# WangFeng18/3d-gaussian-splatting

Hardware: AMD Instinct MI355X
Metric: render_fps (higher is better)
Workload: dtype f32; 1 GPU; cfg5: 2400000 Gaussians, 1920x1080, no SH, forward render, one frame in flight, one view per GPU -- north-star target scene (geometry of BASELINE configs[3]/[4]); n_gaussians=2400000, visible=1887982, tile_pairs=6950364, width=1920, height=1080, parallelism=view-sharded x1 (no data-path collective), frames_in_flight=1

## Files before the change

### 3d-gaussian-splatting_amd/csrc/cull_project.hip

```cpp
#include <atomic>
#include <mutex>

#include "gs_common.h"
#include "gs_frame_layout.h"
#include "project_common.h"
#include "strip_common.h"
#include "tile_bin_common.h"

namespace {

__global__ void __launch_bounds__(256) global_culling_kernel(
    const float *__restrict__ pos, const float4 *__restrict__ quat, const float *__restrict__ scale,
    const float *__restrict__ rot, const float *__restrict__ tran, int64_t n, float near_plane,
    float half_w, float half_h, float *__restrict__ res_pos, float4 *__restrict__ res_cov,
    int64_t *__restrict__ mask) {
    Cam cam;
#pragma unroll
    for (int i = 0; i < 9; ++i) cam.rot[i] = rot[i];
#pragma unroll
    for (int i = 0; i < 3; ++i) cam.tran[i] = tran[i];
    for (int64_t pid = (int64_t)blockIdx.x * blockDim.x + threadIdx.x; pid < n;
         pid += (int64_t)gridDim.x * blockDim.x) {
        float p[3], s[3], pi[3], cv[4];
        load3(pos, pid, p);
// ... 170 lines not shown
    vis = 0;
    cxy = make_float2(0.f, 0.f);
    uint2 rc = make_uint2(0, 0);
    float depth = 0.f;
    if (project_cull(in.p, P.cam, P.near_plane, P.half_w, P.half_h, pc, pi)) {
        project_cov_static(pc, in.RSSR, P.cam, pi, cv);
        vis = 1;
        uint32_t y0, y1, x0, x1;
        cnt = P.cull_method == 0 ? dist_rect(pi[0], pi[1], P, y0, y1, x0, x1)
                                 : tile_rect(pi[0], pi[1], cv, P, y0, y1, x0, x1);
        rc = make_uint2(y0 | (y1 << 16), x0 | (x1 << 16));
        depth = pi[2];
        cxy = make_float2(pi[0], pi[1]);
        const float4 col = make_float4(in.col[0], in.col[1], in.col[2], 0.0f);
        float cA = 0.f, cB = 0.f, cC = 0.f;
        gs_conic(cv[0], cv[1], cv[2], cv[3], cA, cB, cC);
        float4 *rec = rec_geom + pid * GS_REC_STRIDE;
        rec[0] = make_float4(pi[0], pi[1], pi[2], in.opa_act);
        rec[1] = make_float4(cv[0], cv[1], cv[2], cv[3]);
        rec[2] = col;
        rec[3] = make_float4(cA, cB, cC, 0.f);
    }
    if (tiles_touched) tiles_touched[pid] = cnt;
    const uint4 out = make_uint4(rc.x, rc.y, __float_as_uint(depth), cnt);
    rects[pid] = out;
    return out;
}
__device__ __forceinline__ uint4 project_one(const RawGaussian &in, int64_t pid, const ProjectParams &P,
                                             float4 *__restrict__ rec_geom, uint32_t *__restrict__ tiles_touched,
                                             uint4 *__restrict__ rects, uint32_t &vis, float2 &cxy) {
    return project_one(make_static(in, P.scale_act, P.color_dim), pid, P, rec_geom, tiles_touched, rects, vis, cxy);
}

__global__ void __launch_bounds__(256) scene_pack_build_kernel(
    const float *__restrict__ pos, const float4 *__restrict__ quat, const float *__restrict__ scale,
    const float *__restrict__ opa, const float *__restrict__ rgb, int64_t n, int scale_act, int color_dim,
    float4 *__restrict__ pack_a, float4 *__restrict__ pack_b) {
    for (int64_t pid = (int64_t)blockIdx.x * blockDim.x + threadIdx.x; pid < n; pid += (int64_t)gridDim.x * blockDim.x) {
        float s[3];
        const StaticGaussian g = make_static(load_raw(pos, quat, scale, opa, rgb, pid, color_dim), scale_act, color_dim, s);
        float smax = fmaxf(s[0], fmaxf(s[1], s[2]));
        if (!(s[0] + s[1] + s[2] < 3.0e38f)) smax = __uint_as_float(0x7fc00000u);
        pack_a[pid] = make_float4(g.p[0], g.p[1], g.p[2], smax);
        store_static(pack_b, pid, g);
    }
}

__global__ void __launch_bounds__(256) frame_project_kernel(
    const float *__restrict__ pos, const float4 *__restrict__ quat, const float *__restrict__ scale,
    const float *__restrict__ opa, const float *__restrict__ rgb, int64_t n, ProjectParams P,
    float4 *__restrict__ rec_geom,
    uint32_t *__restrict__ tiles_touched, uint4 *__restrict__ rects, uint32_t *__restrict__ block_sums,
    uint32_t *__restrict__ block_vis) {
    const int64_t pid = (int64_t)blockIdx.x * blockDim.x + threadIdx.x;
    uint32_t cnt = 0, vis = 0;
    if (pid < n) {
        float2 cxy;
        cnt = project_one(load_raw(pos, quat, scale, opa, rgb, pid, P.color_dim), pid, P, rec_geom, tiles_touched, rects,
                          vis, cxy).w;
    }
    __shared__ uint32_t s_cnt[4], s_vis[4];
    uint32_t wsum = gs_wave_sum_u32(cnt), wvis = gs_wave_sum_u32(vis);
    const int wave = threadIdx.x >> 6;
    if ((threadIdx.x & 63) == 0) {
        s_cnt[wave] = wsum;
        s_vis[wave] = wvis;
    }
    __syncthreads();
    if (threadIdx.x == 0) {
        block_sums[blockIdx.x] = s_cnt[0] + s_cnt[1] + s_cnt[2] + s_cnt[3];
        block_vis[blockIdx.x] = s_vis[0] + s_vis[1] + s_vis[2] + s_vis[3];
    }
}

template <bool DIST, bool PACKED>
__device__ __forceinline__ void project_count_body(
    const float *__restrict__ pos, const float4 *__restrict__ quat, const float *__restrict__ scale,
    const float *__restrict__ opa, const float *__restrict__ rgb, const float4 *__restrict__ pack_b, int64_t n, ProjectParams P,
    float4 *__restrict__ rec_geom, uint32_t *__restrict__ tiles_touched, uint4 *__restrict__ rects, GsDistCull D,
    uint32_t per_slice, gs_strip_geom SG, uint32_t S, uint32_t slice0, unsigned long long *__restrict__ table,
    uint32_t *__restrict__ slice_pairs, uint32_t *__restrict__ slice_vis, const uint32_t *__restrict__ tile_cost,
    uint32_t n_tiles, uint32_t *__restrict__ tile_order, const unsigned long long *__restrict__ gate) {
    extern __shared__ unsigned long long s_hist[];
    __shared__ uint32_t s_acc[2];
    if (gate && *gate == 0) return;
    if (blockIdx.x >= S) {
        tile_order_workgroup(tile_cost, n_tiles, tile_order);
        return;
    }
    const uint32_t slice = slice0 + strip_slice_of_block(blockIdx.x, S);
    const int64_t g0 = (int64_t)slice * per_slice;
    auto in_range = [&](uint32_t i) { return i < per_slice && g0 + i < n; };
    auto load = [&](int64_t pid) {
        if constexpr (PACKED) return load_static(pack_b, pid);
        else return load_raw(pos, quat, scale, opa, rgb, pid, P.color_dim);
    };
    decltype(load(0)) cur = {}, nxt = {};
    if (in_range(threadIdx.x)) cur = load(g0 + threadIdx.x);
    for (uint32_t t = threadIdx.x; t < SG.NS; t += STRIP_THREADS) s_hist[t] = 0;
    if (threadIdx.x < 2) s_acc[threadIdx.x] = 0;
    __syncthreads();
    settle(cur);
    uint32_t acc_cnt = 0, acc_vis = 0;
    for (uint32_t base = 0; base < per_slice; base += STRIP_THREADS) {
        const uint32_t i = base + threadIdx.x;
        if (in_range(i + STRIP_THREADS)) nxt = load(g0 + i + STRIP_THREADS);
        uint4 rc = make_uint4(0, 0, 0, 0);
        uint32_t vis = 0;
        float2 cxy = make_float2(0.f, 0.f);
        if (in_range(i)) rc = project_one(cur, g0 + i, P, rec_geom, tiles_touched, rects, vis, cxy);
        acc_cnt += rc.w;
        acc_vis += vis;
        walk_strips<DIST>(rc, g0 + i, SG, cxy, D,
                          [&](uint32_t strip, uint32_t, uint32_t, uint32_t np) { atomicAdd(&s_hist[strip], (1ull << 32) | np); });
        cur = nxt;
    }
    acc_cnt = gs_wave_sum_u32(acc_cnt);
    acc_vis = gs_wave_sum_u32(acc_vis);
    if ((threadIdx.x & 63) == 0) {
        atomicAdd(&s_acc[0], acc_cnt);
        atomicAdd(&s_acc[1], acc_vis);
    }
    __syncthreads();
    unsigned long long *row = table + (size_t)slice * SG.NS;
    for (uint32_t t = threadIdx.x; t < SG.NS; t += STRIP_THREADS) row[t] = s_hist[t];
    if (threadIdx.x == 0) {
        slice_pairs[slice] = s_acc[0];
        slice_vis[slice] = s_acc[1];
    }
}

template <bool DIST>
__global__ void __launch_bounds__(STRIP_THREADS) frame_project_count_kernel(
    const float *__restrict__ pos, const float4 *__restrict__ quat, const float *__restrict__ scale,
    const float *__restrict__ opa, const float *__restrict__ rgb, int64_t n, ProjectParams P,
    float4 *__restrict__ rec_geom, uint32_t *__restrict__ tiles_touched, uint4 *__restrict__ rects, GsDistCull D,
    uint32_t per_slice, gs_strip_geom SG, uint32_t S, uint32_t slice0, unsigned long long *__restrict__ table,
    uint32_t *__restrict__ slice_pairs, uint32_t *__restrict__ slice_vis, const uint32_t *__restrict__ tile_cost,
    uint32_t n_tiles, uint32_t *__restrict__ tile_order, const unsigned long long *__restrict__ gate) {
    project_count_body<DIST, false>(pos, quat, scale, opa, rgb, nullptr, n, P, rec_geom, tiles_touched, rects, D, per_slice, SG, S, slice0, table, slice_pairs, slice_vis,
                                    tile_cost, n_tiles, tile_order, gate);
}
template <bool DIST>
__global__ void __launch_bounds__(STRIP_THREADS) frame_packed_project_count_kernel(
    const float4 *__restrict__ pack_b, int64_t n, ProjectParams P,
    float4 *__restrict__ rec_geom, uint32_t *__restrict__ tiles_touched, uint4 *__restrict__ rects, GsDistCull D,
    uint32_t per_slice, gs_strip_geom SG, uint32_t S, uint32_t slice0, unsigned long long *__restrict__ table,
    uint32_t *__restrict__ slice_pairs, uint32_t *__restrict__ slice_vis, const uint32_t *__restrict__ tile_cost,
    uint32_t n_tiles, uint32_t *__restrict__ tile_order, const unsigned long long *__restrict__ gate) {
    project_count_body<DIST, true>(nullptr, nullptr, nullptr, nullptr, nullptr, pack_b, n, P, rec_geom, tiles_touched, rects, D, per_slice, SG, S, slice0, table, slice_pairs, slice_vis,
                                    tile_cost, n_tiles, tile_order, gate);
}

#define GS_OCC_QCAP 16384u
#define GS_OCC_LEVELS 4
struct OccPyramid {
    const uint32_t *t0;
    uint32_t o1, o2, o3;
    uint32_t st0, d1, d2, d3;
};
__device__ __forceinline__ bool occluded_everywhere(const float pi[3], float z, float smax, uint32_t dbits,
                                                    const ProjectParams &P, const OccPyramid &Y) {
    if (P.cull_method != 2) return false;
    const float k = P.occ_k * smax * gs_rcp(z);
    const float ax = 1.0f + pi[0] * pi[0], ay = 1.0f + pi[1] * pi[1];
    const float rx = k * (ax * gs_rsq(ax)) * 1.0001f, ry = k * (ay * gs_rsq(ay)) * 1.0001f;
    const float fx0 = (pi[0] - rx - P.leftmost) * P.inv_tlx - 1e-3f, fx1 = (pi[0] + rx - P.leftmost) * P.inv_tlx + 1e-3f;
    const float fy0 = (pi[1] - ry - P.topmost) * P.inv_tly - 1e-3f, fy1 = (pi[1] + ry - P.topmost) * P.inv_tly + 1e-3f;
    if (!(fx1 - fx0 < 16.0f) || !(fy1 - fy0 < 16.0f)) return false;
    if (fx1 < 0.f || fy1 < 0.f) return true;
    uint32_t x0 = gs_f2u_sat(fx0), y0 = gs_f2u_sat(fy0), x1 = gs_f2u_sat(fx1), y1 = gs_f2u_sat(fy1);
    if (x0 >= P.ntx || y0 >= P.nty) return true;
    x1 = x1 < P.ntx ? x1 : P.ntx - 1;
    y1 = y1 < P.nty ? y1 : P.nty - 1;
    const uint32_t e = (x1 - x0) > (y1 - y0) ? (x1 - x0) : (y1 - y0);
    const uint32_t L = e <= 1 ? 0u : (e <= 3 ? 1u : (e <= 7 ? 2u : 3u));
    const uint32_t m1 = L >= 1 ? ~0u : 0u, m2 = L >= 2 ? ~0u : 0u, m3 = L >= 3 ? ~0u : 0u;
    const uint32_t *tab = Y.t0 + ((Y.o1 & m1) + (Y.o2 & m2) + (Y.o3 & m3));
    const uint32_t st = Y.st0 + ((Y.d1 & m1) + (Y.d2 & m2) + (Y.d3 & m3));
    const uint32_t cx0 = x0 >> L, cy0 = y0 >> L, w = (x1 >> L) - cx0, h = (y1 >> L) - cy0;
    uint32_t m = 0;
#pragma unroll
    for (uint32_t j = 0; j < 3; ++j)
#pragma unroll
        for (uint32_t i = 0; i < 3; ++i) {
            const uint32_t c = tab[(cy0 + (j < h ? j : h)) * st + cx0 + (i < w ? i : w)];
            m = c > m ? c : m;
        }
    return dbits > m;
}

template <bool PACKED>
__device__ __forceinline__ void project_cull_count_body(
    const float *__restrict__ pos, const float4 *__restrict__ quat, const float *__restrict__ scale,
    const float *__restrict__ opa, const float *__restrict__ rgb, const float4 *__restrict__ pack_a,
    const float4 *__restrict__ pack_b, int64_t n, ProjectParams P,
    float4 *__restrict__ rec_geom, uint4 *__restrict__ rects, uint32_t per_slice, gs_strip_geom SG, uint32_t S,
    unsigned long long *__restrict__ table, uint32_t *__restrict__ slice_pairs, uint32_t *__restrict__ slice_vis,
    const uint32_t *__restrict__ tile_cost, uint32_t n_tiles, uint32_t *__restrict__ tile_order,
    const uint32_t *__restrict__ cut, uint32_t qcap, uint32_t stash_cap, unsigned long long *__restrict__ stage_ent,
    uint32_t *__restrict__ stage_tag, uint32_t ecap, uint32_t *__restrict__ slice_entries) {
    extern __shared__ unsigned long long s_hist[];
    __shared__ uint32_t s_acc[2], s_qn, s_ne;
    if (blockIdx.x >= S) {
        tile_order_workgroup(tile_cost, n_tiles, tile_order);
        return;
    }
    const uint32_t slice = strip_slice_of_block(blockIdx.x, S);
    const int64_t g0 = (int64_t)slice * per_slice;
    const int lane = threadIdx.x & 63;
    uint32_t *s_cut = reinterpret_cast<uint32_t *>(s_hist + SG.NS);
    const uint32_t st0 = SG.nsx * GS_STRIP_W;
    const uint32_t w1 = (SG.ntx + 1) / 2, h1 = (SG.nty + 1) / 2, w2 = (w1 + 1) / 2, h2 = (h1 + 1) / 2, w3 = (w2 + 1) / 2,
                   h3 = (h2 + 1) / 2;
    uint32_t *s_l1 = s_cut + st0 * SG.nty, *s_l2 = s_l1 + w1 * h1, *s_l3 = s_l2 + w2 * h2;
    uint16_t *s_q = reinterpret_cast<uint16_t *>(s_l3 + w3 * h3);
    float *s_stash = reinterpret_cast<float *>(s_q + ((qcap + 1) & ~1u));
    const OccPyramid Y = {s_cut, st0 * SG.nty, w1 * h1, w2 * h2, st0, w1 - st0, w2 - w1, w3 - w2};
    auto fetch_at = [&](float (&pp)[3], float (&ss)[3], uint32_t i) {
        int64_t g = g0 + i;
        g = g < n ? g : n - 1;
        if constexpr (PACKED) {
            const float4 v = pack_a[g];
            pp[0] = v.x; pp[1] = v.y; pp[2] = v.z; ss[0] = v.w;
            ss[1] = ss[2] = 0.f;
        } else {
            load3(pos, g, pp);
            load3(scale, g, ss);
        }
    };
    float pa[3], sa[3], pb[3], sb[3];
    fetch_at(pa, sa, threadIdx.x);
    fetch_at(pb, sb, threadIdx.x + STRIP_THREADS);
    for (uint32_t t = threadIdx.x; t < SG.NS; t += STRIP_THREADS) s_hist[t] = 0;
    for (uint32_t t0 = threadIdx.x; t0 < st0 * SG.nty; t0 += 8 * STRIP_THREADS) {
        uint32_t v[8];
#pragma unroll
        for (uint32_t k = 0; k < 8; ++k) {
            const uint32_t t = t0 + k * STRIP_THREADS, iy = t / st0, ix = t - iy * st0;
            const bool in = iy < SG.nty && ix < SG.ntx;
            v[k] = cut[in ? iy * SG.ntx + ix : 0u];
            v[k] = in ? v[k] : GS_NO_CUT;
        }
#pragma unroll
        for (uint32_t k = 0; k < 8; ++k)
            if (t0 + k * STRIP_THREADS < st0 * SG.nty) s_cut[t0 + k * STRIP_THREADS] = v[k];
    }
    if (threadIdx.x < 2) s_acc[threadIdx.x] = 0;
    if (threadIdx.x == 2) s_ne = 0;
    unsigned long long *const ent = stage_ent + (size_t)slice * ecap;
    uint32_t *const tag = stage_tag + (size_t)slice * ecap;
    auto build = [&](uint32_t *dst, uint32_t dw, uint32_t dh, const uint32_t *src, uint32_t sst, uint32_t sw, uint32_t sh) {
        __syncthreads();
        for (uint32_t t = threadIdx.x; t < dw * dh; t += STRIP_THREADS) {
            const uint32_t cy = t / dw, cx = t - cy * dw, x = 2 * cx, y = 2 * cy;
            uint32_t m = src[y * sst + x];
            if (x + 1 < sw) m = max(m, src[y * sst + x + 1]);
            if (y + 1 < sh) {
                m = max(m, src[(y + 1) * sst + x]);
                if (x + 1 < sw) m = max(m, src[(y + 1) * sst + x + 1]);
            }
            dst[t] = m;
        }
    };
    build(s_l1, w1, h1, s_cut, st0, SG.ntx, SG.nty);
    build(s_l2, w2, h2, s_l1, w1, w1, h1);
    build(s_l3, w3, h3, s_l2, w2, w2, h2);
    uint32_t acc_cnt = 0, acc_vis = 0;
    for (uint32_t c0 = 0; c0 < per_slice; c0 += qcap) {
        const uint32_t cn = per_slice - c0 < qcap ? per_slice - c0 : qcap;
        if (threadIdx.x == 0) s_qn = 0;
        __syncthreads();
        auto in_chunk = [&](uint32_t i) { return i < cn && g0 + c0 + i < n; };
        auto fetch = [&](float (&pp)[3], float (&ss)[3], uint32_t i) { fetch_at(pp, ss, c0 + i); };
        auto test = [&](const float (&pp)[3], const float (&ss)[3], uint32_t i) {
            bool surv = false;
            if (in_chunk(i)) {
                float pc[3], pi[3];
                if (project_cull(pp, P.cam, P.near_plane, P.half_w, P.half_h, pc, pi)) {
                    const float dep = sqrtf(pc[0] * pc[0] + pc[1] * pc[1] + pc[2] * pc[2]);
                    float smax;
                    bool finite;
                    if constexpr (PACKED) {
                        smax = ss[0];
                        finite = smax < 3.0e38f;
                    } else {
                        float s[3];
#pragma unroll
                        for (int k = 0; k < 3; ++k) s[k] = P.scale_act == 0 ? fabsf(ss[k]) + 1e-4f : gs_exp2(GS_LOG2E * ss[k]);
                        smax = fmaxf(s[0], fmaxf(s[1], s[2]));
                        finite = s[0] + s[1] + s[2] < 3.0e38f;
                    }
                    if (finite && occluded_everywhere(pi, pc[2], smax, __float_as_uint(dep), P, Y)) {
                        acc_vis += 1;
                    } else {
                        surv = true;
                    }
                }
            }
            const unsigned long long b = __ballot(surv);
            if (b) {
                uint32_t wbase = 0;
                if (lane == 0) wbase = atomicAdd(&s_qn, (uint32_t)__popcll(b));
                wbase = __shfl(wbase, 0, 64);
                if (surv) {
                    const uint32_t slot = wbase + (uint32_t)__popcll(b & ((1ull << lane) - 1ull));
                    s_q[slot] = (uint16_t)i;
                    if (!PACKED && slot < stash_cap) {
#pragma unroll
                        for (int c = 0; c < 3; ++c) {
                            s_stash[c * stash_cap + slot] = pp[c];
                            s_stash[(3 + c) * stash_cap + slot] = ss[c];
                        }
                    }
                }
            }
        };
        float pq[3], sq[3];
        if (c0 != 0) {
            fetch(pa, sa, threadIdx.x);
            fetch(pb, sb, threadIdx.x + STRIP_THREADS);
        }
        for (uint32_t base = 0; base < cn; base += 3 * STRIP_THREADS) {
            const uint32_t i = base + threadIdx.x;
            fetch(pq, sq, i + 2 * STRIP_THREADS);
            test(pa, sa, i);
            if (base + STRIP_THREADS >= cn) break;
            fetch(pa, sa, i + 3 * STRIP_THREADS);
            test(pb, sb, i + STRIP_THREADS);
            if (base + 2 * STRIP_THREADS >= cn) break;
            fetch(pb, sb, i + 4 * STRIP_THREADS);
            test(pq, sq, i + 2 * STRIP_THREADS);
        }
        __syncthreads();
        const uint32_t nq = s_qn;
        auto load_survivor = [&](uint32_t k, uint32_t q) {
            const int64_t pid = g0 + c0 + q;
            if constexpr (PACKED) {
                return load_static(pack_b, pid);
            } else {
                RawGaussian r;
                if (k < stash_cap) {
#pragma unroll
                    for (int c = 0; c < 3; ++c) {
                        r.p[c] = s_stash[c * stash_cap + k];
                        r.sraw[c] = s_stash[(3 + c) * stash_cap + k];
                    }
                } else {
                    load3(pos, pid, r.p);
                    load3(scale, pid, r.sraw);
                }
                const float4 q4 = quat[pid];
                r.qraw[0] = q4.x; r.qraw[1] = q4.y; r.qraw[2] = q4.z; r.qraw[3] = q4.w;
                r.opa = opa[pid];
                r.rgb[0] = r.rgb[1] = r.rgb[2] = 0.f;
                if (P.color_dim == 3) load3(rgb, pid, r.rgb);
                return r;
            }
        };
        decltype(load_survivor(0, 0)) cur = {}, nxt = {};
        uint32_t qi = 0, qn_ = 0;
        if (threadIdx.x < nq) {
            qi = s_q[threadIdx.x];
            cur = load_survivor(threadIdx.x, qi);
        }
        settle(cur);
        for (uint32_t base = 0; base < nq; base += STRIP_THREADS) {
            const uint32_t k = base + threadIdx.x;
            if (k + STRIP_THREADS < nq) {
                qn_ = s_q[k + STRIP_THREADS];
                nxt = load_survivor(k + STRIP_THREADS, qn_);
            }
            uint4 rc = make_uint4(0, 0, 0, 0);
            uint32_t vis = 0;
            float2 cxy = make_float2(0.f, 0.f);
            const int64_t pid = g0 + c0 + qi;
            if (k < nq) rc = project_one(cur, pid, P, rec_geom, nullptr, rects, vis, cxy);
            acc_cnt += rc.w;
            acc_vis += vis;
            walk_strips<false, true>(rc, pid, SG, cxy, GsDistCull{},
                                     [&](uint32_t strip, uint32_t lo32, uint32_t d, uint32_t np) {
                                         const uint32_t rank = (uint32_t)(atomicAdd(&s_hist[strip], (1ull << 32) | np) >> 32);
                                         const unsigned long long act = __ballot(true);
                                         uint32_t wbase = 0;
                                         if (lane == __ffsll((long long)act) - 1) wbase = atomicAdd(&s_ne, (uint32_t)__popcll(act));
                                         wbase = (uint32_t)__builtin_amdgcn_readfirstlane((int)wbase);
                                         const uint32_t slot = wbase + (uint32_t)__popcll(act & ((1ull << lane) - 1ull));
                                         if (slot < ecap) {
                                             ent[slot] = ((unsigned long long)d << 32) | lo32;
                                             tag[slot] = strip_tag(strip, rank);
                                         }
                                     },
                                     s_cut);
            cur = nxt;
            qi = qn_;
        }
    }
    acc_cnt = gs_wave_sum_u32(acc_cnt);
    acc_vis = gs_wave_sum_u32(acc_vis);
    if (lane == 0) {
        atomicAdd(&s_acc[0], acc_cnt);
        atomicAdd(&s_acc[1], acc_vis);
    }
    __syncthreads();
    const uint32_t ne = s_ne;
    const bool fits = ne <= ecap;
    unsigned long long *row = table + (size_t)slice * SG.NS;
    for (uint32_t t = threadIdx.x; t < SG.NS; t += STRIP_THREADS) row[t] = fits ? s_hist[t] : 0ull;
    if (threadIdx.x == 0) {
        slice_pairs[slice] = s_acc[0];
        slice_vis[slice] = s_acc[1];
        slice_entries[slice] = fits ? ne : GS_STAGE_OVER;
    }
}

__global__ void __launch_bounds__(STRIP_THREADS) frame_project_cull_count_kernel(
    const float *__restrict__ pos, const float4 *__restrict__ quat, const float *__restrict__ scale,
    const float *__restrict__ opa, const float *__restrict__ rgb, int64_t n, ProjectParams P,
    float4 *__restrict__ rec_geom, uint4 *__restrict__ rects, uint32_t per_slice, gs_strip_geom SG, uint32_t S,
    unsigned long long *__restrict__ table, uint32_t *__restrict__ slice_pairs, uint32_t *__restrict__ slice_vis,
    const uint32_t *__restrict__ tile_cost, uint32_t n_tiles, uint32_t *__restrict__ tile_order,
    const uint32_t *__restrict__ cut, uint32_t qcap, uint32_t stash_cap, unsigned long long *__restrict__ stage_ent,
    uint32_t *__restrict__ stage_tag, uint32_t ecap, uint32_t *__restrict__ slice_entries) {
    project_cull_count_body<false>(pos, quat, scale, opa, rgb, nullptr, nullptr, n, P, rec_geom, rects, per_slice, SG, S, table, slice_pairs, slice_vis, tile_cost, n_tiles, tile_order, cut,
                                   qcap, stash_cap, stage_ent, stage_tag, ecap, slice_entries);
}
__global__ void __launch_bounds__(STRIP_THREADS) frame_packed_project_cull_count_kernel(
    const float4 *__restrict__ pack_a, const float4 *__restrict__ pack_b, int64_t n, ProjectParams P,
    float4 *__restrict__ rec_geom, uint4 *__restrict__ rects, uint32_t per_slice, gs_strip_geom SG, uint32_t S,
    unsigned long long *__restrict__ table, uint32_t *__restrict__ slice_pairs, uint32_t *__restrict__ slice_vis,
    const uint32_t *__restrict__ tile_cost, uint32_t n_tiles, uint32_t *__restrict__ tile_order,
    const uint32_t *__restrict__ cut, uint32_t qcap, uint32_t stash_cap, unsigned long long *__restrict__ stage_ent,
    uint32_t *__restrict__ stage_tag, uint32_t ecap, uint32_t *__restrict__ slice_entries) {
    project_cull_count_body<true>(nullptr, nullptr, nullptr, nullptr, nullptr, pack_a, pack_b, n, P, rec_geom, rects, per_slice, SG, S, table, slice_pairs, slice_vis, tile_cost, n_tiles, tile_order, cut,
                                   qcap, stash_cap, stage_ent, stage_tag, ecap, slice_entries);
}

template <bool DIST>
__global__ void __launch_bounds__(BIN_THREADS) frame_project_bin_count_kernel(
    const float *__restrict__ pos, const float4 *__restrict__ quat, const float *__restrict__ scale,
    const float *__restrict__ opa, const float *__restrict__ rgb, int64_t n, ProjectParams P,
    float4 *__restrict__ rec_geom, uint4 *__restrict__ rects, GsDistCull D, uint32_t per_block, uint32_t T,
    uint32_t *__restrict__ table, uint32_t *__restrict__ slice_pairs, uint32_t *__restrict__ slice_vis) {
    extern __shared__ uint32_t s_tile_hist[];
    __shared__ uint32_t s_acc[2];
    const uint32_t slice = slice_of_block(blockIdx.x, gridDim.x);
    const int64_t g0 = (int64_t)slice * per_block;
    auto in_range = [&](uint32_t i) { return i < per_block && g0 + i < n; };
    RawGaussian cur = {}, nxt = {};
    if (in_range(threadIdx.x)) cur = load_raw(pos, quat, scale, opa, rgb, g0 + threadIdx.x, P.color_dim);
    for (uint32_t t = threadIdx.x; t < T; t += BIN_THREADS) s_tile_hist[t] = 0;
    if (threadIdx.x < 2) s_acc[threadIdx.x] = 0;
    __syncthreads();
    settle(cur);
    uint32_t acc_cnt = 0, acc_vis = 0;
    for (uint32_t base = 0; base < per_block; base += BIN_THREADS) {
        const uint32_t i = base + threadIdx.x;
        if (in_range(i + BIN_THREADS)) nxt = load_raw(pos, quat, scale, opa, rgb, g0 + i + BIN_THREADS, P.color_dim);
        uint4 rc = make_uint4(0, 0, 0, 0);
        uint32_t vis = 0;
        float2 cxy = make_float2(0.f, 0.f);
        if (in_range(i)) rc = project_one(cur, g0 + i, P, rec_geom, nullptr, rects, vis, cxy);
        acc_cnt += rc.w;
        acc_vis += vis;
        walk_rect<DIST>(rc, g0 + i, P.ntx, cxy, D, [&](uint32_t tile, uint32_t, uint32_t) { atomicAdd(&s_tile_hist[tile], 1u); });
        cur = nxt;
    }
    acc_cnt = gs_wave_sum_u32(acc_cnt);
    acc_vis = gs_wave_sum_u32(acc_vis);
    if ((threadIdx.x & 63) == 0) {
        atomicAdd(&s_acc[0], acc_cnt);
        atomicAdd(&s_acc[1], acc_vis);
    }
    __syncthreads();
    uint32_t *row = table + (size_t)slice * T;
    for (uint32_t t = threadIdx.x; t < T; t += BIN_THREADS) row[t] = s_tile_hist[t];
    if (threadIdx.x == 0) {
        slice_pairs[slice] = s_acc[0];
        slice_vis[slice] = s_acc[1];
    }
}

}

extern "C" int gs_world2camera(const float *pos, const float *rot, const float *tran, float *res, int64_t B,
                               gs_stream_t stream) {
    GS_CHECK_ARG(B >= 0, "B < 0");
    if (B == 0) return 0;
    GS_CHECK_ARG(pos && rot && tran && res, "null pointer");
    hipLaunchKernelGGL(world2camera_kernel, dim3(grid_for(B, 256)), dim3(256), 0, (hipStream_t)stream, pos, rot,
                       tran, res, B);
    GS_CHECK_LAUNCH();
    return 0;
}

extern "C" int gs_world2camera_backward(const float *grad_out, const float *rot, float *grad_inp, int64_t B,
                                        gs_stream_t stream) {
    GS_CHECK_ARG(B >= 0, "B < 0");
    if (B == 0) return 0;
    GS_CHECK_ARG(grad_out && rot && grad_inp, "null pointer");
    hipLaunchKernelGGL(world2camera_backward_kernel, dim3(grid_for(B, 256)), dim3(256), 0, (hipStream_t)stream,
                       grad_out, rot, grad_inp, B);
    GS_CHECK_LAUNCH();
    return 0;
}

extern "C" int gs_jacobian(const float *pos_cam, float *jac, int64_t B, gs_stream_t stream) {
    GS_CHECK_ARG(B >= 0, "B < 0");
    if (B == 0) return 0;
    GS_CHECK_ARG(pos_cam && jac, "null pointer");
    hipLaunchKernelGGL(jacobian_kernel, dim3(grid_for(B, 256)), dim3(256), 0, (hipStream_t)stream, pos_cam, jac, B);
    GS_CHECK_LAUNCH();
    return 0;
}

extern "C" int gs_global_culling(const float *pos, const float *quat, const float *scale, const float *rot,
                                 const float *tran, int64_t N, float near_plane, float half_width,
                                 float half_height, float *res_pos, float *res_cov, int64_t *culling_mask,
                                 gs_stream_t stream) {
    GS_CHECK_ARG(N >= 0, "N < 0");
    if (N == 0) return 0;
    GS_CHECK_ARG(pos && quat && scale && rot && tran && res_pos && res_cov && culling_mask, "null pointer");
    GS_CHECK_ARG(((uintptr_t)quat & 15) == 0 && ((uintptr_t)res_cov & 15) == 0, "quat/res_cov must be 16-byte aligned");
    hipLaunchKernelGGL(global_culling_kernel, dim3(grid_for(N, 256)), dim3(256), 0, (hipStream_t)stream, pos,
                       (const float4 *)quat, scale, rot, tran, N, near_plane, half_width, half_height, res_pos,
                       (float4 *)res_cov, culling_mask);
    GS_CHECK_LAUNCH();
    return 0;
}

extern "C" size_t gs_scene_pack_bytes(int64_t N, size_t *a_bytes, size_t *b_bytes) {
    const size_t a = N < 0 ? 0 : ((size_t)N * 16 + 255) / 256 * 256, b = N < 0 ? 0 : ((size_t)N * 64 + 255) / 256 * 256;
    if (a_bytes) *a_bytes = a;
    if (b_bytes) *b_bytes = b;
    return a + b;
}

extern "C" int gs_scene_pack_build(const float *pos, const float *quat, const float *scale, const float *opa, const float *rgb,
                                   int64_t N, int32_t color_dim, int32_t scale_activation, void *pack_a, void *pack_b,
                                   gs_stream_t stream) {
    GS_CHECK_ARG(N >= 0 && N < (1ll << 31), "N out of range");
    GS_CHECK_ARG(color_dim == 3 || color_dim == 27 || color_dim == 48, "color_dim must be 3, 27 or 48");
    GS_CHECK_ARG(scale_activation == 0 || scale_activation == 1, "scale_activation must be 0 (abs) or 1 (exp)");
    if (N == 0) return 0;
    GS_CHECK_ARG(pos && quat && scale && opa && rgb && pack_a && pack_b, "null pointer");
    GS_CHECK_ARG(((uintptr_t)quat & 15) == 0, "quat must be 16-byte aligned");
    GS_CHECK_ARG(((uintptr_t)pack_a & 15) == 0 && ((uintptr_t)pack_b & 63) == 0,
                 "pack_a must be 16-byte aligned, pack_b 64-byte aligned");
    hipLaunchKernelGGL(scene_pack_build_kernel, dim3(grid_for(N, 256)), dim3(256), 0, (hipStream_t)stream, pos,
                       (const float4 *)quat, scale, opa, rgb, N, (int)scale_activation, (int)color_dim, (float4 *)pack_a,
                       (float4 *)pack_b);
    GS_CHECK_LAUNCH();
    return 0;
}

int gs_stage_project(const gs_frame *f, const gs_frame_ws &ws, hipStream_t stream, int slice_begin, int slice_end,
                     bool second_pass) {
    ProjectParams P = make_params(f);
    uint32_t *touched = f->sort_mode == 2 && gs_frame_geometry(f).n_tiles <= GS_BIN_MAX_TILES ? nullptr : ws.tiles_touched;
    if (gs_frame_uses_strips(f)) {
        touched = nullptr;
        gs_frame_geom G = gs_frame_geometry(f);
        const gs_strip_plan plan = gs_strip_plan_for(f->N, G.ntx, G.nty);
        const gs_strip_geom SG = plan.geom;
        const GsDistCull D = gs_frame_dist_cull(f);
        static std::mutex attr_mu;
        static std::atomic<uint64_t> attr_done{0};
        int dev = 0;
        GS_HIP(hipGetDevice(&dev));
        if (dev < 64 && !((attr_done.load(std::memory_order_acquire) >> dev) & 1)) {
            std::lock_guard<std::mutex> lock(attr_mu);
            for (const void *fn : {(const void *)frame_project_count_kernel<false>, (const void *)frame_project_count_kernel<true>,
                                   (const void *)frame_packed_project_count_kernel<false>, (const void *)frame_packed_project_count_kernel<true>,
                                   (const void *)frame_project_cull_count_kernel, (const void *)frame_packed_project_cull_count_kernel})
                GS_HIP(hipFuncSetAttribute(fn, hipFuncAttributeMaxDynamicSharedMemorySize, GS_BIN_LDS_BYTES - 8 * 4096));
            attr_done.fetch_or(1ull << dev, std::memory_order_release);
        }
        unsigned long long *table = (unsigned long long *)ws.strip_table;
        if (slice_end < 0) slice_end = (int)plan.slices;
        GS_CHECK_ARG(slice_begin >= 0 && slice_begin < slice_end && slice_end <= (int)plan.slices, "bad slice range");
        const uint32_t nsl = (uint32_t)(slice_end - slice_begin);
        const bool packed = gs_frame_scene_pack(f);
        const float4 *pack_a = packed ? (const float4 *)gs_frame_scene_fields(f)->scene_pack_a : nullptr;
        const float4 *pack_b = packed ? (const float4 *)gs_frame_scene_fields(f)->scene_pack_b : nullptr;
        if (gs_frame_occlusion_cull(f) && !second_pass) {
            GS_CHECK_ARG(slice_begin == 0 && nsl == plan.slices, "an occlusion-culled frame is projected in one piece");
            uint32_t qcap_max = GS_OCC_QCAP;
            if (const char *e = getenv("GS_OCC_QCAP")) {
                const long v = atol(e);
                if (v >= 64 && v <= (long)GS_OCC_QCAP) qcap_max = (uint32_t)v;
            }
            const uint32_t qcap = plan.per_slice < qcap_max ? plan.per_slice : qcap_max;
            size_t lds = sizeof(unsigned long long) * SG.NS + gs_cull_pyramid_bytes(G.ntx, G.nty) + 2 * (size_t)qcap + 16;
            const size_t room = (size_t)GS_BIN_LDS_BYTES - 8 * 4096;
            uint32_t stash_cap = room > lds ? (uint32_t)((room - lds) / 24) & ~63u : 0u;
            if (stash_cap > qcap) stash_cap = (qcap + 63u) & ~63u;
            if (packed) stash_cap = 0;
            if (const char *e = getenv("GS_OCC_STASH")) {
                const long v = atol(e);
                if (v >= 0 && (uint32_t)v < stash_cap) stash_cap = (uint32_t)v & ~63u;
            }
            lds += (size_t)stash_cap * 24;
#define GS_CULL_TAIL                                                                                                   \
    f->N, P, ws.rec_geom, ws.rects, plan.per_slice, SG, nsl, table, ws.slice_pairs, ws.slice_vis, ws.tile_cost,        \
        (uint32_t)G.n_tiles, ws.tile_order, gs_frame_cut_table(f, ws), qcap, stash_cap, (unsigned long long *)ws.keys_b, \
        ws.vals_b, gs_cull_stage_cap(f->max_pairs, plan.slices), ws.slice_entries
            if (packed)
                hipLaunchKernelGGL(frame_packed_project_cull_count_kernel, dim3(nsl + 1), dim3(STRIP_THREADS), lds, stream, pack_a,
                                   pack_b, GS_CULL_TAIL);
            else
                hipLaunchKernelGGL(frame_project_cull_count_kernel, dim3(nsl + 1), dim3(STRIP_THREADS), lds, stream, f->pos,
                                   (const float4 *)f->quat, f->scale, f->opa, f->rgb, GS_CULL_TAIL);
#undef GS_CULL_TAIL
            GS_CHECK_LAUNCH();
            return 0;
        }
        const size_t lds = sizeof(unsigned long long) * SG.NS;
        const uint32_t extra = (slice_begin == 0 && !second_pass) ? 1u : 0u;
        const unsigned long long *gate = second_pass ? ws.counters + GS_CNT_RANPAST : nullptr;
#define GS_COUNT_TAIL                                                                                                  \
    f->N, P, ws.rec_geom, touched, ws.rects, D, plan.per_slice, SG, nsl, (uint32_t)slice_begin, table, ws.slice_pairs, \
        ws.slice_vis, ws.tile_cost, (uint32_t)G.n_tiles, ws.tile_order, gate
#define GS_LAUNCH_PROJECT_COUNT(DIST)                                                                                  \
    do {                                                                                                               \
        if (packed)                                                                                                    \
            hipLaunchKernelGGL(frame_packed_project_count_kernel<DIST>, dim3(nsl + extra), dim3(STRIP_THREADS), lds,   \
                               stream, pack_b, GS_COUNT_TAIL);                                                         \
        else                                                                                                           \
            hipLaunchKernelGGL(frame_project_count_kernel<DIST>, dim3(nsl + extra), dim3(STRIP_THREADS), lds, stream,  \
                               f->pos, (const float4 *)f->quat, f->scale, f->opa, f->rgb, GS_COUNT_TAIL);              \
    } while (0)
        if (f->tile_culling_method == 0)
            GS_LAUNCH_PROJECT_COUNT(true);
        else
            GS_LAUNCH_PROJECT_COUNT(false);
#undef GS_LAUNCH_PROJECT_COUNT
#undef GS_COUNT_TAIL
        GS_CHECK_LAUNCH();
        return 0;
    }
    GS_CHECK_ARG(!second_pass, "the second pass of an occlusion-culled frame belongs to the strip variant's project + count stage");
    GS_CHECK_ARG(slice_begin == 0 && slice_end < 0, "this frame's project stage cannot be issued in ranges");
    if (gs_frame_fused_table_count(f)) {
        gs_frame_geom G = gs_frame_geometry(f);
        const GsDistCull D = gs_frame_dist_cull(f);
        static std::mutex attr_mu2;
        static std::atomic<uint64_t> attr_done2{0};
        int dev = 0;
        GS_HIP(hipGetDevice(&dev));
        if (dev < 64 && !((attr_done2.load(std::memory_order_acquire) >> dev) & 1)) {
            std::lock_guard<std::mutex> lock(attr_mu2);
            for (const void *fn : {(const void *)frame_project_bin_count_kernel<false>, (const void *)frame_project_bin_count_kernel<true>})
                GS_HIP(hipFuncSetAttribute(fn, hipFuncAttributeMaxDynamicSharedMemorySize, GS_BIN_MAX_TILES * 4));
            attr_done2.fetch_or(1ull << dev, std::memory_order_release);
        }
        const uint32_t per_block = bin_per_block(f->N), B = (uint32_t)gs_div_up(f->N, per_block);
        const uint32_t T = (uint32_t)G.n_tiles;
#define GS_LAUNCH_PROJECT_BIN(DIST)                                                                                    \
    hipLaunchKernelGGL(frame_project_bin_count_kernel<DIST>, dim3(B), dim3(BIN_THREADS), sizeof(uint32_t) * T, stream, \
                       f->pos, (const float4 *)f->quat, f->scale, f->opa, f->rgb, f->N, P, ws.rec_geom, ws.rects, D,   \
                       per_block, T, ws.bin_table, ws.slice_pairs, ws.slice_vis)
        if (f->tile_culling_method == 0)
            GS_LAUNCH_PROJECT_BIN(true);
        else
            GS_LAUNCH_PROJECT_BIN(false);
#undef GS_LAUNCH_PROJECT_BIN
        GS_CHECK_LAUNCH();
        return 0;
    }
    int nblk = (int)gs_div_up(f->N, 256);
    hipLaunchKernelGGL(frame_project_kernel, dim3(nblk), dim3(256), 0, stream, f->pos, (const float4 *)f->quat,
                       f->scale, f->opa, f->rgb, f->N, P, ws.rec_geom,
                       touched, ws.rects, ws.block_sums, ws.block_vis);
    GS_CHECK_LAUNCH();
    return 0;
}
```

Measured before the change: 4507 frames/s.

## Stream occlusion-cull survivors through per-wave LDS rings instead of chunked block queue

Replaces the chunked two-phase scheme, where a block tests a chunk, syncs, then projects the queued survivors, with a per-wavefront ring buffer in LDS. Each wave projects 64 survivors as soon as they accumulate, interleaved with culling the next candidates, and leftovers go to a shared tail list that is handled after a single block barrier. The goal is to remove block-wide barriers and idle phases and to overlap cull tests with projection. In exchange, each wave needs its own small parameter stash, sizing becomes more intricate, and correctness depends on ordering the ring within a wavefront.

```diff
diff --git a/3d-gaussian-splatting_amd/csrc/cull_project.hip b/3d-gaussian-splatting_amd/csrc/cull_project.hip
--- a/3d-gaussian-splatting_amd/csrc/cull_project.hip
+++ b/3d-gaussian-splatting_amd/csrc/cull_project.hip
@@ -346,7 +346,6 @@
                                     tile_cost, n_tiles, tile_order, gate);
 }
 
-#define GS_OCC_QCAP 16384u
 #define GS_OCC_LEVELS 4
 struct OccPyramid {
     const uint32_t *t0;
@@ -384,6 +383,9 @@
     return dbits > m;
 }
 
+#define GS_OCC_RING 128u
+#define GS_OCC_TAIL (16u * 63u)
+
 template <bool PACKED>
 __device__ __forceinline__ void project_cull_count_body(
     const float *__restrict__ pos, const float4 *__restrict__ quat, const float *__restrict__ scale,
@@ -392,26 +394,27 @@
     float4 *__restrict__ rec_geom, uint4 *__restrict__ rects, uint32_t per_slice, gs_strip_geom SG, uint32_t S,
     unsigned long long *__restrict__ table, uint32_t *__restrict__ slice_pairs, uint32_t *__restrict__ slice_vis,
     const uint32_t *__restrict__ tile_cost, uint32_t n_tiles, uint32_t *__restrict__ tile_order,
-    const uint32_t *__restrict__ cut, uint32_t qcap, uint32_t stash_cap, unsigned long long *__restrict__ stage_ent,
+    const uint32_t *__restrict__ cut, uint32_t par_slots, unsigned long long *__restrict__ stage_ent,
     uint32_t *__restrict__ stage_tag, uint32_t ecap, uint32_t *__restrict__ slice_entries) {
     extern __shared__ unsigned long long s_hist[];
-    __shared__ uint32_t s_acc[2], s_qn, s_ne;
+    __shared__ uint32_t s_acc[2], s_tn, s_ne;
     if (blockIdx.x >= S) {
         tile_order_workgroup(tile_cost, n_tiles, tile_order);
         return;
     }
     const uint32_t slice = strip_slice_of_block(blockIdx.x, S);
     const int64_t g0 = (int64_t)slice * per_slice;
-    const int lane = threadIdx.x & 63;
+    const uint32_t lane = threadIdx.x & 63, wave = threadIdx.x >> 6;
     uint32_t *s_cut = reinterpret_cast<uint32_t *>(s_hist + SG.NS);
     const uint32_t st0 = SG.nsx * GS_STRIP_W;
     const uint32_t w1 = (SG.ntx + 1) / 2, h1 = (SG.nty + 1) / 2, w2 = (w1 + 1) / 2, h2 = (h1 + 1) / 2, w3 = (w2 + 1) / 2,
                    h3 = (h2 + 1) / 2;
     uint32_t *s_l1 = s_cut + st0 * SG.nty, *s_l2 = s_l1 + w1 * h1, *s_l3 = s_l2 + w2 * h2;
-    uint16_t *s_q = reinterpret_cast<uint16_t *>(s_l3 + w3 * h3);
-    float *s_stash = reinterpret_cast<float *>(s_q + ((qcap + 1) & ~1u));
+    uint32_t *s_tail = s_l3 + w3 * h3 + (STRIP_THREADS / 64) * GS_OCC_RING;
+    uint32_t *const ring = s_l3 + w3 * h3 + wave * GS_OCC_RING;
+    float *const par = reinterpret_cast<float *>(s_tail + GS_OCC_TAIL) + wave * 6 * par_slots;
     const OccPyramid Y = {s_cut, st0 * SG.nty, w1 * h1, w2 * h2, st0, w1 - st0, w2 - w1, w3 - w2};
-    auto fetch_at = [&](float (&pp)[3], float (&ss)[3], uint32_t i) {
+    auto fetch = [&](float (&pp)[3], float (&ss)[3], uint32_t i) {
         int64_t g = g0 + i;
         g = g < n ? g : n - 1;
         if constexpr (PACKED) {
@@ -424,8 +427,8 @@
         }
     };
     float pa[3], sa[3], pb[3], sb[3];
-    fetch_at(pa, sa, threadIdx.x);
-    fetch_at(pb, sb, threadIdx.x + STRIP_THREADS);
+    fetch(pa, sa, threadIdx.x);
+    fetch(pb, sb, threadIdx.x + STRIP_THREADS);
     for (uint32_t t = threadIdx.x; t < SG.NS; t += STRIP_THREADS) s_hist[t] = 0;
     for (uint32_t t0 = threadIdx.x; t0 < st0 * SG.nty; t0 += 8 * STRIP_THREADS) {
         uint32_t v[8];
@@ -442,6 +445,7 @@
     }
     if (threadIdx.x < 2) s_acc[threadIdx.x] = 0;
     if (threadIdx.x == 2) s_ne = 0;
+    if (threadIdx.x == 3) s_tn = 0;
     unsigned long long *const ent = stage_ent + (size_t)slice * ecap;
     uint32_t *const tag = stage_tag + (size_t)slice * ecap;
     auto build = [&](uint32_t *dst, uint32_t dw, uint32_t dh, const uint32_t *src, uint32_t sst, uint32_t sw, uint32_t sh) {
@@ -460,134 +464,168 @@
     build(s_l1, w1, h1, s_cut, st0, SG.ntx, SG.nty);
     build(s_l2, w2, h2, s_l1, w1, w1, h1);
     build(s_l3, w3, h3, s_l2, w2, w2, h2);
+    __syncthreads();
     uint32_t acc_cnt = 0, acc_vis = 0;
-    for (uint32_t c0 = 0; c0 < per_slice; c0 += qcap) {
-        const uint32_t cn = per_slice - c0 < qcap ? per_slice - c0 : qcap;
-        if (threadIdx.x == 0) s_qn = 0;
-        __syncthreads();
-        auto in_chunk = [&](uint32_t i) { return i < cn && g0 + c0 + i < n; };
-        auto fetch = [&](float (&pp)[3], float (&ss)[3], uint32_t i) { fetch_at(pp, ss, c0 + i); };
-        auto test = [&](const float (&pp)[3], const float (&ss)[3], uint32_t i) {
-            bool surv = false;
-            if (in_chunk(i)) {
-                float pc[3], pi[3];
-                if (project_cull(pp, P.cam, P.near_plane, P.half_w, P.half_h, pc, pi)) {
-                    const float dep = sqrtf(pc[0] * pc[0] + pc[1] * pc[1] + pc[2] * pc[2]);
-                    float smax;
-                    bool finite;
-                    if constexpr (PACKED) {
-                        smax = ss[0];
-                        finite = smax < 3.0e38f;
-                    } else {
-                        float s[3];
+    uint32_t head = 0, tail = 0;
+    auto ring_order = [] {
+        __builtin_amdgcn_fence(__ATOMIC_ACQ_REL, "wavefront");
+        __builtin_amdgcn_wave_barrier();
+    };
+    auto in_slice = [&](uint32_t i) { return i < per_slice && g0 + i < n; };
+    auto test = [&](const float (&pp)[3], const float (&ss)[3], uint32_t i) {
+        bool surv = false;
+        if (in_slice(i)) {
+            float pc[3], pi[3];
+            if (project_cull(pp, P.cam, P.near_plane, P.half_w, P.half_h, pc, pi)) {
+                const float dep = sqrtf(pc[0] * pc[0] + pc[1] * pc[1] + pc[2] * pc[2]);
+                float smax;
+                bool finite;
+                if constexpr (PACKED) {
+                    smax = ss[0];
+                    finite = smax < 3.0e38f;
+                } else {
+                    float s[3];
 #pragma unroll
-                        for (int k = 0; k < 3; ++k) s[k] = P.scale_act == 0 ? fabsf(ss[k]) + 1e-4f : gs_exp2(GS_LOG2E * ss[k]);
-                        smax = fmaxf(s[0], fmaxf(s[1], s[2]));
-                        finite = s[0] + s[1] + s[2] < 3.0e38f;
-                    }
-                    if (finite && occluded_everywhere(pi, pc[2], smax, __float_as_uint(dep), P, Y)) {
-                        acc_vis += 1;
-                    } else {
-                        surv = true;
-                    }
+                    for (int k = 0; k < 3; ++k) s[k] = P.scale_act == 0 ? fabsf(ss[k]) + 1e-4f : gs_exp2(GS_LOG2E * ss[k]);
+                    smax = fmaxf(s[0], fmaxf(s[1], s[2]));
+                    finite = s[0] + s[1] + s[2] < 3.0e38f;
+                }
+                if (finite && occluded_everywhere(pi, pc[2], smax, __float_as_uint(dep), P, Y)) {
+                    acc_vis += 1;
+                } else {
+                    surv = true;
                 }
             }
-            const unsigned long long b = __ballot(surv);
-            if (b) {
-                uint32_t wbase = 0;
-                if (lane == 0) wbase = atomicAdd(&s_qn, (uint32_t)__popcll(b));
-                wbase = __shfl(wbase, 0, 64);
-                if (surv) {
-                    const uint32_t slot = wbase + (uint32_t)__popcll(b & ((1ull << lane) - 1ull));
-                    s_q[slot] = (uint16_t)i;
-                    if (!PACKED && slot < stash_cap) {
+        }
+        const unsigned long long b = __ballot(surv);
+        if (surv) {
+            const uint32_t below = __builtin_amdgcn_mbcnt_hi((uint32_t)(b >> 32), __builtin_amdgcn_mbcnt_lo((uint32_t)b, 0u));
+            const uint32_t slot = (tail + below) & (GS_OCC_RING - 1);
+            ring[slot] = i;
+            if (!PACKED && slot < par_slots) {
 #pragma unroll
-                        for (int c = 0; c < 3; ++c) {
-                            s_stash[c * stash_cap + slot] = pp[c];
-                            s_stash[(3 + c) * stash_cap + slot] = ss[c];
-                        }
-                    }
+                for (int c = 0; c < 3; ++c) {
+                    par[c * par_slots + slot] = pp[c];
+                    par[(3 + c) * par_slots + slot] = ss[c];
                 }
             }
-        };
-        float pq[3], sq[3];
-        if (c0 != 0) {
-            fetch(pa, sa, threadIdx.x);
-            fetch(pb, sb, threadIdx.x + STRIP_THREADS);
-        }
-        for (uint32_t base = 0; base < cn; base += 3 * STRIP_THREADS) {
-            const uint32_t i = base + threadIdx.x;
-            fetch(pq, sq, i + 2 * STRIP_THREADS);
-            test(pa, sa, i);
-            if (base + STRIP_THREADS >= cn) break;
-            fetch(pa, sa, i + 3 * STRIP_THREADS);
-            test(pb, sb, i + STRIP_THREADS);
-            if (base + 2 * STRIP_THREADS >= cn) break;
-            fetch(pb, sb, i + 4 * STRIP_THREADS);
-            test(pq, sq, i + 2 * STRIP_THREADS);
-        }
-        __syncthreads();
-        const uint32_t nq = s_qn;
-        auto load_survivor = [&](uint32_t k, uint32_t q) {
-            const int64_t pid = g0 + c0 + q;
-            if constexpr (PACKED) {
-                return load_static(pack_b, pid);
+        }
+        tail += (uint32_t)__popcll(b);
+    };
+    auto load_survivor = [&](uint32_t slot, uint32_t q) {
+        const int64_t pid = g0 + q;
+        if constexpr (PACKED) {
+            return load_static(pack_b, pid);
+        } else {
+            RawGaussian r;
+            if (slot < par_slots) {
+#pragma unroll
+                for (int c = 0; c < 3; ++c) {
+                    r.p[c] = par[c * par_slots + slot];
+                    r.sraw[c] = par[(3 + c) * par_slots + slot];
+                }
             } else {
-                RawGaussian r;
-                if (k < stash_cap) {
-#pragma unroll
-                    for (int c = 0; c < 3; ++c) {
-                        r.p[c] = s_stash[c * stash_cap + k];
-                        r.sraw[c] = s_stash[(3 + c) * stash_cap + k];
-                    }
-                } else {
-                    load3(pos, pid, r.p);
-                    load3(scale, pid, r.sraw);
-                }
-                const float4 q4 = quat[pid];
-                r.qraw[0] = q4.x; r.qraw[1] = q4.y; r.qraw[2] = q4.z; r.qraw[3] = q4.w;
-                r.opa = opa[pid];
-                r.rgb[0] = r.rgb[1] = r.rgb[2] = 0.f;
-                if (P.color_dim == 3) load3(rgb, pid, r.rgb);
-                return r;
+                load3(pos, pid, r.p);
+                load3(scale, pid, r.sraw);
             }
-        };
-        decltype(load_survivor(0, 0)) cur = {}, nxt = {};
-        uint32_t qi = 0, qn_ = 0;
-        if (threadIdx.x < nq) {
-            qi = s_q[threadIdx.x];
-            cur = load_survivor(threadIdx.x, qi);
-        }
-        settle(cur);
-        for (uint32_t base = 0; base < nq; base += STRIP_THREADS) {
-            const uint32_t k = base + threadIdx.x;
-            if (k + STRIP_THREADS < nq) {
-                qn_ = s_q[k + STRIP_THREADS];
-                nxt = load_survivor(k + STRIP_THREADS, qn_);
-            }
-            uint4 rc = make_uint4(0, 0, 0, 0);
-            uint32_t vis = 0;
-            float2 cxy = make_float2(0.f, 0.f);
-            const int64_t pid = g0 + c0 + qi;
-            if (k < nq) rc = project_one(cur, pid, P, rec_geom, nullptr, rects, vis, cxy);
-            acc_cnt += rc.w;
-            acc_vis += vis;
-            walk_strips<false, true>(rc, pid, SG, cxy, GsDistCull{},
-                                     [&](uint32_t strip, uint32_t lo32, uint32_t d, uint32_t np) {
-                                         const uint32_t rank = (uint32_t)(atomicAdd(&s_hist[strip], (1ull << 32) | np) >> 32);
-                                         const unsigned long long act = __ballot(true);
-                                         uint32_t wbase = 0;
-                                         if (lane == __ffsll((long long)act) - 1) wbase = atomicAdd(&s_ne, (uint32_t)__popcll(act));
-                                         wbase = (uint32_t)__builtin_amdgcn_readfirstlane((int)wbase);
-                                         const uint32_t slot = wbase + (uint32_t)__popcll(act & ((1ull << lane) - 1ull));
-                                         if (slot < ecap) {
-                                             ent[slot] = ((unsigned long long)d << 32) | lo32;
-                                             tag[slot] = strip_tag(strip, rank);
-                                         }
-                                     },
-                                     s_cut);
-            cur = nxt;
-            qi = qn_;
+            const float4 q4 = quat[pid];
+            r.qraw[0] = q4.x; r.qraw[1] = q4.y; r.qraw[2] = q4.z; r.qraw[3] = q4.w;
+            r.opa = opa[pid];
+            r.rgb[0] = r.rgb[1] = r.rgb[2] = 0.f;
+            if (P.color_dim == 3) load3(rgb, pid, r.rgb);
+            return r;
+        }
+    };
+    using Survivor = decltype(load_survivor(0, 0));
+    auto project_walk = [&](const Survivor &g, uint32_t q, bool active) {
+        uint4 rc = make_uint4(0, 0, 0, 0);
+        uint32_t vis = 0;
+        float2 cxy = make_float2(0.f, 0.f);
+        const int64_t pid = g0 + q;
+        if (active) rc = project_one(g, pid, P, rec_geom, nullptr, rects, vis, cxy);
+        acc_cnt += rc.w;
+        acc_vis += vis;
+        walk_strips<false, true>(rc, pid, SG, cxy, GsDistCull{},
+                                 [&](uint32_t strip, uint32_t lo32, uint32_t d, uint32_t np) {
+                                     const uint32_t rank = (uint32_t)(atomicAdd(&s_hist[strip], (1ull << 32) | np) >> 32);
+                                     const unsigned long long act = __ballot(true);
+                                     uint32_t wbase = 0;
+                                     if ((int)lane == __ffsll((long long)act) - 1) wbase = atomicAdd(&s_ne, (uint32_t)__popcll(act));
+                                     wbase = (uint32_t)__builtin_amdgcn_readfirstlane((int)wbase);
+                                     const uint32_t slot = wbase + (uint32_t)__popcll(act & ((1ull << lane) - 1ull));
+                                     if (slot < ecap) {
+                                         ent[slot] = ((unsigned long long)d << 32) | lo32;
+                                         tag[slot] = strip_tag(strip, rank);
+                                     }
+                                 },
+                                 s_cut);
+    };
+    Survivor cur = {};
+    uint32_t qi = 0;
+    bool pending = false;
+    auto request = [&] {
+        if (tail - head >= 64u) {
+            ring_order();
+            const uint32_t slot = (head + lane) & (GS_OCC_RING - 1);
+            qi = ring[slot];
+            ring_order();
+            head += 64u;
+            cur = load_survivor(slot, qi);
+            pending = true;
+        }
+    };
+    auto finish = [&] {
+        if (pending) {
+            project_walk(cur, qi, true);
+            pending = false;
+        }
+    };
+    auto settle_set = [&](const float (&pp)[3], const float (&ss)[3]) {
+        if constexpr (PACKED) asm volatile("" ::"v"(pp[0]), "v"(pp[1]), "v"(pp[2]), "v"(ss[0]));
+        else asm volatile("" ::"v"(pp[0]), "v"(pp[1]), "v"(pp[2]), "v"(ss[0]), "v"(ss[1]), "v"(ss[2]));
+    };
+    float pq[3], sq[3];
+    for (uint32_t base = 0; base < per_slice; base += 3 * STRIP_THREADS) {
+        const uint32_t i = base + threadIdx.x;
+        fetch(pq, sq, i + 2 * STRIP_THREADS);
+        test(pa, sa, i);
+        settle_set(pb, sb);
+        finish();
+        request();
+        if (base + STRIP_THREADS >= per_slice) break;
+        fetch(pa, sa, i + 3 * STRIP_THREADS);
+        test(pb, sb, i + STRIP_THREADS);
+        settle_set(pq, sq);
+        finish();
+        request();
+        if (base + 2 * STRIP_THREADS >= per_slice) break;
+        fetch(pb, sb, i + 4 * STRIP_THREADS);
+        test(pq, sq, i + 2 * STRIP_THREADS);
+        settle_set(pa, sa);
+        finish();
+        request();
+    }
+    finish();
+    {
+        const uint32_t left = tail - head;
+        uint32_t tbase = 0;
+        if (left) {
+            if (lane == 0) tbase = atomicAdd(&s_tn, left);
+            tbase = (uint32_t)__builtin_amdgcn_readfirstlane((int)tbase);
+            ring_order();
+            if (lane < left) s_tail[tbase + lane] = ring[(head + lane) & (GS_OCC_RING - 1)];
+        }
+    }
+    __syncthreads();
+    {
+        const uint32_t nt = s_tn;
+        if (wave * 64u < nt) {
+            const uint32_t k = threadIdx.x;
+            const bool active = k < nt;
+            const uint32_t q = active ? s_tail[k] : 0u;
+            Survivor g = {};
+            if (active) g = load_survivor(GS_OCC_RING, q);
+            project_walk(g, q, active);
         }
     }
     acc_cnt = gs_wave_sum_u32(acc_cnt);
@@ -614,20 +652,20 @@
     float4 *__restrict__ rec_geom, uint4 *__restrict__ rects, uint32_t per_slice, gs_strip_geom SG, uint32_t S,
     unsigned long long *__restrict__ table, uint32_t *__restrict__ slice_pairs, uint32_t *__restrict__ slice_vis,
     const uint32_t *__restrict__ tile_cost, uint32_t n_tiles, uint32_t *__restrict__ tile_order,
-    const uint32_t *__restrict__ cut, uint32_t qcap, uint32_t stash_cap, unsigned long long *__restrict__ stage_ent,
+    const uint32_t *__restrict__ cut, uint32_t par_slots, unsigned long long *__restrict__ stage_ent,
     uint32_t *__restrict__ stage_tag, uint32_t ecap, uint32_t *__restrict__ slice_entries) {
     project_cull_count_body<false>(pos, quat, scale, opa, rgb, nullptr, nullptr, n, P, rec_geom, rects, per_slice, SG, S, table, slice_pairs, slice_vis, tile_cost, n_tiles, tile_order, cut,
-                                   qcap, stash_cap, stage_ent, stage_tag, ecap, slice_entries);
+                                   par_slots, stage_ent, stage_tag, ecap, slice_entries);
 }
 __global__ void __launch_bounds__(STRIP_THREADS) frame_packed_project_cull_count_kernel(
     const float4 *__restrict__ pack_a, const float4 *__restrict__ pack_b, int64_t n, ProjectParams P,
     float4 *__restrict__ rec_geom, uint4 *__restrict__ rects, uint32_t per_slice, gs_strip_geom SG, uint32_t S,
     unsigned long long *__restrict__ table, uint32_t *__restrict__ slice_pairs, uint32_t *__restrict__ slice_vis,
     const uint32_t *__restrict__ tile_cost, uint32_t n_tiles, uint32_t *__restrict__ tile_order,
-    const uint32_t *__restrict__ cut, uint32_t qcap, uint32_t stash_cap, unsigned long long *__restrict__ stage_ent,
+    const uint32_t *__restrict__ cut, uint32_t par_slots, unsigned long long *__restrict__ stage_ent,
     uint32_t *__restrict__ stage_tag, uint32_t ecap, uint32_t *__restrict__ slice_entries) {
     project_cull_count_body<true>(nullptr, nullptr, nullptr, nullptr, nullptr, pack_a, pack_b, n, P, rec_geom, rects, per_slice, SG, S, table, slice_pairs, slice_vis, tile_cost, n_tiles, tile_order, cut,
-                                   qcap, stash_cap, stage_ent, stage_tag, ecap, slice_entries);
+                                   par_slots, stage_ent, stage_tag, ecap, slice_entries);
 }
 
 template <bool DIST>
@@ -779,25 +817,20 @@
         const float4 *pack_b = packed ? (const float4 *)gs_frame_scene_fields(f)->scene_pack_b : nullptr;
         if (gs_frame_occlusion_cull(f) && !second_pass) {
             GS_CHECK_ARG(slice_begin == 0 && nsl == plan.slices, "an occlusion-culled frame is projected in one piece");
-            uint32_t qcap_max = GS_OCC_QCAP;
-            if (const char *e = getenv("GS_OCC_QCAP")) {
-                const long v = atol(e);
-                if (v >= 64 && v <= (long)GS_OCC_QCAP) qcap_max = (uint32_t)v;
-            }
-            const uint32_t qcap = plan.per_slice < qcap_max ? plan.per_slice : qcap_max;
-            size_t lds = sizeof(unsigned long long) * SG.NS + gs_cull_pyramid_bytes(G.ntx, G.nty) + 2 * (size_t)qcap + 16;
+            size_t lds = sizeof(unsigned long long) * SG.NS + gs_cull_pyramid_bytes(G.ntx, G.nty) +
+                         sizeof(uint32_t) * ((STRIP_THREADS / 64) * GS_OCC_RING + GS_OCC_TAIL);
             const size_t room = (size_t)GS_BIN_LDS_BYTES - 8 * 4096;
-            uint32_t stash_cap = room > lds ? (uint32_t)((room - lds) / 24) & ~63u : 0u;
-            if (stash_cap > qcap) stash_cap = (qcap + 63u) & ~63u;
-            if (packed) stash_cap = 0;
+            uint32_t par_slots = room > lds ? (uint32_t)((room - lds) / (24 * (STRIP_THREADS / 64))) : 0u;
+            if (par_slots > GS_OCC_RING) par_slots = GS_OCC_RING;
+            if (packed) par_slots = 0;
             if (const char *e = getenv("GS_OCC_STASH")) {
                 const long v = atol(e);
-                if (v >= 0 && (uint32_t)v < stash_cap) stash_cap = (uint32_t)v & ~63u;
+                if (v >= 0 && (uint32_t)(v / (STRIP_THREADS / 64)) < par_slots) par_slots = (uint32_t)(v / (STRIP_THREADS / 64));
             }
-            lds += (size_t)stash_cap * 24;
+            lds += (size_t)par_slots * 24 * (STRIP_THREADS / 64);
 #define GS_CULL_TAIL                                                                                                   \
     f->N, P, ws.rec_geom, ws.rects, plan.per_slice, SG, nsl, table, ws.slice_pairs, ws.slice_vis, ws.tile_cost,        \
-        (uint32_t)G.n_tiles, ws.tile_order, gs_frame_cut_table(f, ws), qcap, stash_cap, (unsigned long long *)ws.keys_b, \
+        (uint32_t)G.n_tiles, ws.tile_order, gs_frame_cut_table(f, ws), par_slots, (unsigned long long *)ws.keys_b,       \
         ws.vals_b, gs_cull_stage_cap(f->max_pairs, plan.slices), ws.slice_entries
             if (packed)
                 hipLaunchKernelGGL(frame_packed_project_cull_count_kernel, dim3(nsl + 1), dim3(STRIP_THREADS), lds, stream, pack_a,
```

After: 4630 frames/s (median of 6 runs). 2.7% higher.
